# omerbt/TokenFlow

Hardware: NVIDIA H100
Metric: frames/sec for 40-frame 512x512 SD1.5 50-step edit (higher is better)
Workload: dtype fp16

## Files before the change

### tokenflow_b200/csrc/tf_nn_field.cu

```cuda
#include <cmath>

#include "tf_common.cuh"
#include "tf_kernels.h"
#include "tf_wgmma.cuh"

namespace tf {
namespace {

constexpr int kChunkK = 64;
constexpr int kBlockM = 128;
constexpr int kBlockN = 128;
constexpr int kMaxStages = 8;
constexpr int kSmemBudget = 227 * 1024;

struct NNItems {
  int32_t n_a;
  int32_t n_b;
  int32_t tiles_per_frame;
  int32_t n_b_frames;
  int32_t b_frames[kMaxFrames];
};

struct SmemCtl {
  uint64_t full[kMaxStages];
  uint64_t empty[kMaxStages];
  uint64_t a_full;
};

template <bool kResidentA>
__global__ void __launch_bounds__(288, 1)
nn_field_kernel(const __grid_constant__ CUtensorMap map_x, const __grid_constant__ CUtensorMap map_p,
                const FrameTable tab, const NNItems items, int S, int dim, int stages,
                int32_t* __restrict__ idx_a, int32_t* __restrict__ idx_b) {
  constexpr int kAChunkBytes = kBlockM * 128;
  constexpr int kBChunkBytes = kBlockN * 128;
  constexpr int kStageBytes = kBChunkBytes + (kResidentA ? 0 : kAChunkBytes);
  constexpr int kAcc = kBlockN / 2;

  extern __shared__ uint8_t smem_raw[];
  uint8_t* smem = reinterpret_cast<uint8_t*>((reinterpret_cast<uintptr_t>(smem_raw) + 1023) & ~uintptr_t(1023));
  const int nkc = (dim + kChunkK - 1) / kChunkK;
  uint8_t* a_res = smem;
  uint8_t* ring = smem + (kResidentA ? nkc * kAChunkBytes : 0);
  SmemCtl* ctl = reinterpret_cast<SmemCtl*>(ring + stages * kStageBytes);

  int f, m0, kf;
  int32_t* out;
  if ((int)blockIdx.x < items.n_a) {
    f = blockIdx.x / items.tiles_per_frame;
    m0 = (blockIdx.x - f * items.tiles_per_frame) * kBlockM;
    kf = tab.kf_a[f];
    out = idx_a;
  } else {
    const int j = blockIdx.x - items.n_a;
    const int fi = j / items.tiles_per_frame;
    f = items.b_frames[fi];
    m0 = (j - fi * items.tiles_per_frame) * kBlockM;
    kf = tab.kf_b[f];
    out = idx_b;
  }
  const int n_tiles = (S + kBlockN - 1) / kBlockN;
  const int J = n_tiles * nkc;

  auto load = [&](int j) {
    const int st = j % stages;
    const int nt = j / nkc, kc = j - nt * nkc;
    uint8_t* dst = ring + st * kStageBytes;
    mbar_arrive_expect_tx(&ctl->full[st], (uint32_t)kStageBytes);
    tma_load_3d(dst, &map_p, &ctl->full[st], kc * kChunkK, nt * kBlockN, kf);
    if (!kResidentA) tma_load_3d(dst + kBChunkBytes, &map_x, &ctl->full[st], kc * kChunkK, m0, f);
  };

  if (threadIdx.x == 0) {
    tma_prefetch_desc(&map_x);
    tma_prefetch_desc(&map_p);
    for (int i = 0; i < stages; ++i) {
      mbar_init(&ctl->full[i], 1);
      mbar_init(&ctl->empty[i], 8);
    }
    mbar_init(&ctl->a_full, 1);
    fence_mbar_init();
  }
  __syncthreads();
  if (threadIdx.x >= 256) {
    if (threadIdx.x == 256) {
      if (kResidentA) {
        mbar_arrive_expect_tx(&ctl->a_full, (uint32_t)(nkc * kAChunkBytes));
        for (int kc = 0; kc < nkc; ++kc) tma_load_3d(a_res + kc * kAChunkBytes, &map_x, &ctl->a_full, kc * kChunkK, m0, f);
      }
      for (int j = 0; j < J; ++j) {
        if (j >= stages) mbar_wait(&ctl->empty[j % stages], (uint32_t)(j / stages - 1) & 1u);
        load(j);
      }
    }
    return;
  }

  const int wg = threadIdx.x >> 7;
  const int lane = threadIdx.x & 31;
  const int qcol = 2 * (lane & 3);
  const uint32_t ring_addr = smem_u32(ring);
  const uint32_t a_res_addr = smem_u32(a_res) + wg * 64 * 128;
  if (kResidentA) {
    mbar_wait(&ctl->a_full, 0);
    __syncwarp();
  }

  auto release = [&](int j) {
    __syncwarp();
    if (lane == 0) mbar_arrive(&ctl->empty[j % stages]);
  };

  float best[2] = {-INFINITY, -INFINITY};
  int best_idx[2] = {0, 0};
  int j = 0;
  for (int nt = 0; nt < n_tiles; ++nt) {
    float acc[kAcc];
    for (int kc = 0; kc < nkc; ++kc, ++j) {
      const int st = j % stages;
      mbar_wait(&ctl->full[st], (uint32_t)(j / stages) & 1u);
      __syncwarp();
      const uint32_t b_addr = ring_addr + st * kStageBytes;
      const uint32_t a_addr = kResidentA ? a_res_addr + kc * kAChunkBytes : b_addr + kBChunkBytes + wg * 64 * 128;
      wgmma_fence();
#pragma unroll
      for (int k4 = 0; k4 < kChunkK / 16; ++k4)
        wgmma_ss<kBlockN>(acc, wgmma_desc(a_addr + k4 * 32, 16, 1024), wgmma_desc(b_addr + k4 * 32, 16, 1024),
                          (kc > 0 || k4 > 0) ? 1u : 0u);
      wgmma_commit();
      if (kc > 0) {
        wgmma_wait<1>();
        release(j - 1);
      }
    }
    wgmma_wait<0>();
    reg_fence(acc);
    release(j - 1);

    const int n0 = nt * kBlockN;
#pragma unroll
    for (int jb = 0; jb < kBlockN / 8; ++jb) {
#pragma unroll
      for (int e = 0; e < 4; ++e) {
        const int r = e >> 1;
        const int c = n0 + 8 * jb + qcol + (e & 1);
        const float h = __half2float(__float2half_rn(acc[4 * jb + e]));
        if (c < S && h > best[r]) { best[r] = h; best_idx[r] = c; }
      }
    }
  }

#pragma unroll
  for (int r = 0; r < 2; ++r) {
#pragma unroll
    for (int off = 1; off <= 2; off <<= 1) {
      const float ob = __shfl_xor_sync(0xffffffffu, best[r], off);
      const int oi = __shfl_xor_sync(0xffffffffu, best_idx[r], off);
      if (ob > best[r] || (ob == best[r] && oi < best_idx[r])) { best[r] = ob; best_idx[r] = oi; }
    }
    const int p = m0 + wg * 64 + ((threadIdx.x >> 5) & 3) * 16 + (lane >> 2) + 8 * r;
    if ((lane & 3) == 0 && p < S) out[(long long)f * S + p] = best_idx[r];
  }
}

template <bool kResidentA>
int launch_cfg(const void* x_unit, const void* piv_unit, const FrameTable& tab, const NNItems& items, int F, int S,
               int dim, int K, int32_t* idx_a, int32_t* idx_b, cudaStream_t stream) {
  const int nkc = (dim + kChunkK - 1) / kChunkK;
  const int a_bytes = kResidentA ? nkc * kBlockM * 128 : 0;
  const int stage_bytes = kBlockN * 128 + (kResidentA ? 0 : kBlockM * 128);
  int stages = (kSmemBudget - 2048 - a_bytes) / stage_bytes;
  if (stages > kMaxStages) stages = kMaxStages;
  if (stages < 2) {
    set_last_error("tf_nn_field: dim=%d does not fit the resident-A configuration", dim);
    return TF_ERR_UNSUPPORTED;
  }
  const size_t smem_bytes = 1024 + (size_t)a_bytes + (size_t)stages * stage_bytes + sizeof(SmemCtl);

  CUtensorMap map_x, map_p;
  {
    const uint64_t dims[3] = {(uint64_t)dim, (uint64_t)S, (uint64_t)F};
    const uint64_t strides[2] = {(uint64_t)dim * 2, (uint64_t)S * dim * 2};
    const uint32_t box[3] = {(uint32_t)kChunkK, (uint32_t)kBlockM, 1};
    CUresult r = encode_tiled(&map_x, CU_TENSOR_MAP_DATA_TYPE_FLOAT16, 3, x_unit, dims, strides, box,
                              CU_TENSOR_MAP_SWIZZLE_128B);
    if (r != CUDA_SUCCESS) { set_last_error("tf_nn_field: cuTensorMapEncodeTiled(x) failed: %d", (int)r); return TF_ERR_DRIVER; }
  }
  {
    const uint64_t dims[3] = {(uint64_t)dim, (uint64_t)S, (uint64_t)K};
    const uint64_t strides[2] = {(uint64_t)dim * 2, (uint64_t)S * dim * 2};
    const uint32_t box[3] = {(uint32_t)kChunkK, (uint32_t)kBlockN, 1};
    CUresult r = encode_tiled(&map_p, CU_TENSOR_MAP_DATA_TYPE_FLOAT16, 3, piv_unit, dims, strides, box,
                              CU_TENSOR_MAP_SWIZZLE_128B);
    if (r != CUDA_SUCCESS) { set_last_error("tf_nn_field: cuTensorMapEncodeTiled(pivots) failed: %d", (int)r); return TF_ERR_DRIVER; }
  }
  auto kern = nn_field_kernel<kResidentA>;
  if (check_cuda(cudaFuncSetAttribute(kern, cudaFuncAttributeMaxDynamicSharedMemorySize, (int)smem_bytes),
                 "tf_nn_field smem attribute"))
    return TF_ERR_CUDA;
  const int n_items = items.n_a + items.n_b;
  kern<<<n_items, 288, smem_bytes, stream>>>(map_x, map_p, tab, items, S, dim, stages, idx_a, idx_b);
  return check_cuda(cudaGetLastError(), "tf_nn_field launch");
}

}

int launch_nn_field(const void* x_unit, const void* piv_unit, const FrameTable& tab, int F, int S, int dim, int K,
                    int32_t* idx_a, int32_t* idx_b, cudaStream_t stream) {
  if (F == 0 || S == 0) return TF_OK;
  NNItems items;
  items.tiles_per_frame = (S + kBlockM - 1) / kBlockM;
  items.n_a = F * items.tiles_per_frame;
  items.n_b_frames = 0;
  for (int f = 0; f < F; ++f)
    if (tab.kf_b[f] >= 0) items.b_frames[items.n_b_frames++] = f;
  items.n_b = items.n_b_frames * items.tiles_per_frame;
  if (items.n_b > 0 && idx_b == nullptr) {
    set_last_error("tf_nn_field: idx_b is NULL but some frame has a second keyframe");
    return TF_ERR_INVALID_ARGUMENT;
  }
  if (dim <= 640) return launch_cfg<true>(x_unit, piv_unit, tab, items, F, S, dim, K, idx_a, idx_b, stream);
  return launch_cfg<false>(x_unit, piv_unit, tab, items, F, S, dim, K, idx_a, idx_b, stream);
}

}
```

### tokenflow_b200/csrc/tf_wgmma.cuh

```cuda
#pragma once

#include <stdint.h>

namespace tf {

template <int N> __device__ __forceinline__ void wgmma_ss(float (&d)[N / 2], uint64_t a, uint64_t b, uint32_t acc);
template <int N> __device__ __forceinline__ void wgmma_rs(float (&d)[N / 2], const uint32_t (&a)[4], uint64_t b, uint32_t acc);

template <>
__device__ __forceinline__ void wgmma_ss<64>(float (&d)[32], uint64_t a, uint64_t b, uint32_t acc) {
  asm volatile(
      "{\n\t.reg .pred p;\n\t"
      "setp.ne.b32 p, %34, 0;\n\t"
      "wgmma.mma_async.sync.aligned.m64n64k16.f32.f16.f16 "
      "{%0, %1, %2, %3, %4, %5, %6, %7, %8, %9, %10, %11, %12, %13, %14, %15, %16, %17, %18, %19, %20, %21, %22, %23, %24, %25, %26, %27, %28, %29, %30, %31}, "
      "%32, %33, p, 1, 1, 0, 0;\n\t}\n"
      : "+f"(d[0]), "+f"(d[1]), "+f"(d[2]), "+f"(d[3]), "+f"(d[4]), "+f"(d[5]), "+f"(d[6]), "+f"(d[7]),
        "+f"(d[8]), "+f"(d[9]), "+f"(d[10]), "+f"(d[11]), "+f"(d[12]), "+f"(d[13]), "+f"(d[14]), "+f"(d[15]),
        "+f"(d[16]), "+f"(d[17]), "+f"(d[18]), "+f"(d[19]), "+f"(d[20]), "+f"(d[21]), "+f"(d[22]), "+f"(d[23]),
        "+f"(d[24]), "+f"(d[25]), "+f"(d[26]), "+f"(d[27]), "+f"(d[28]), "+f"(d[29]), "+f"(d[30]), "+f"(d[31])
      : "l"(a), "l"(b), "r"(acc));
}

template <>
__device__ __forceinline__ void wgmma_ss<128>(float (&d)[64], uint64_t a, uint64_t b, uint32_t acc) {
  asm volatile(
      "{\n\t.reg .pred p;\n\t"
      "setp.ne.b32 p, %66, 0;\n\t"
      "wgmma.mma_async.sync.aligned.m64n128k16.f32.f16.f16 "
      "{%0, %1, %2, %3, %4, %5, %6, %7, %8, %9, %10, %11, %12, %13, %14, %15, %16, %17, %18, %19, %20, %21, %22, %23, %24, %25, %26, %27, %28, %29, %30, %31, %32, %33, %34, %35, %36, %37, %38, %39, %40, %41, %42, %43, %44, %45, %46, %47, %48, %49, %50, %51, %52, %53, %54, %55, %56, %57, %58, %59, %60, %61, %62, %63}, "
      "%64, %65, p, 1, 1, 0, 0;\n\t}\n"
      : "+f"(d[0]), "+f"(d[1]), "+f"(d[2]), "+f"(d[3]), "+f"(d[4]), "+f"(d[5]), "+f"(d[6]), "+f"(d[7]),
        "+f"(d[8]), "+f"(d[9]), "+f"(d[10]), "+f"(d[11]), "+f"(d[12]), "+f"(d[13]), "+f"(d[14]), "+f"(d[15]),
        "+f"(d[16]), "+f"(d[17]), "+f"(d[18]), "+f"(d[19]), "+f"(d[20]), "+f"(d[21]), "+f"(d[22]), "+f"(d[23]),
        "+f"(d[24]), "+f"(d[25]), "+f"(d[26]), "+f"(d[27]), "+f"(d[28]), "+f"(d[29]), "+f"(d[30]), "+f"(d[31]),
        "+f"(d[32]), "+f"(d[33]), "+f"(d[34]), "+f"(d[35]), "+f"(d[36]), "+f"(d[37]), "+f"(d[38]), "+f"(d[39]),
        "+f"(d[40]), "+f"(d[41]), "+f"(d[42]), "+f"(d[43]), "+f"(d[44]), "+f"(d[45]), "+f"(d[46]), "+f"(d[47]),
        "+f"(d[48]), "+f"(d[49]), "+f"(d[50]), "+f"(d[51]), "+f"(d[52]), "+f"(d[53]), "+f"(d[54]), "+f"(d[55]),
        "+f"(d[56]), "+f"(d[57]), "+f"(d[58]), "+f"(d[59]), "+f"(d[60]), "+f"(d[61]), "+f"(d[62]), "+f"(d[63])
      : "l"(a), "l"(b), "r"(acc));
}

template <>
__device__ __forceinline__ void wgmma_rs<16>(float (&d)[8], const uint32_t (&a)[4], uint64_t b, uint32_t acc) {
  asm volatile(
      "{\n\t.reg .pred p;\n\t"
      "setp.ne.b32 p, %13, 0;\n\t"
      "wgmma.mma_async.sync.aligned.m64n16k16.f32.f16.f16 "
      "{%0, %1, %2, %3, %4, %5, %6, %7}, "
      "{%8, %9, %10, %11}, %12, p, 1, 1, 1;\n\t}\n"
      : "+f"(d[0]), "+f"(d[1]), "+f"(d[2]), "+f"(d[3]), "+f"(d[4]), "+f"(d[5]), "+f"(d[6]), "+f"(d[7])
      : "r"(a[0]), "r"(a[1]), "r"(a[2]), "r"(a[3]), "l"(b), "r"(acc));
}

template <>
__device__ __forceinline__ void wgmma_rs<32>(float (&d)[16], const uint32_t (&a)[4], uint64_t b, uint32_t acc) {
  asm volatile(
      "{\n\t.reg .pred p;\n\t"
      "setp.ne.b32 p, %21, 0;\n\t"
      "wgmma.mma_async.sync.aligned.m64n32k16.f32.f16.f16 "
      "{%0, %1, %2, %3, %4, %5, %6, %7, %8, %9, %10, %11, %12, %13, %14, %15}, "
      "{%16, %17, %18, %19}, %20, p, 1, 1, 1;\n\t}\n"
      : "+f"(d[0]), "+f"(d[1]), "+f"(d[2]), "+f"(d[3]), "+f"(d[4]), "+f"(d[5]), "+f"(d[6]), "+f"(d[7]),
        "+f"(d[8]), "+f"(d[9]), "+f"(d[10]), "+f"(d[11]), "+f"(d[12]), "+f"(d[13]), "+f"(d[14]), "+f"(d[15])
      : "r"(a[0]), "r"(a[1]), "r"(a[2]), "r"(a[3]), "l"(b), "r"(acc));
}

template <>
__device__ __forceinline__ void wgmma_rs<48>(float (&d)[24], const uint32_t (&a)[4], uint64_t b, uint32_t acc) {
  asm volatile(
      "{\n\t.reg .pred p;\n\t"
      "setp.ne.b32 p, %29, 0;\n\t"
      "wgmma.mma_async.sync.aligned.m64n48k16.f32.f16.f16 "
      "{%0, %1, %2, %3, %4, %5, %6, %7, %8, %9, %10, %11, %12, %13, %14, %15, %16, %17, %18, %19, %20, %21, %22, %23}, "
      "{%24, %25, %26, %27}, %28, p, 1, 1, 1;\n\t}\n"
      : "+f"(d[0]), "+f"(d[1]), "+f"(d[2]), "+f"(d[3]), "+f"(d[4]), "+f"(d[5]), "+f"(d[6]), "+f"(d[7]),
        "+f"(d[8]), "+f"(d[9]), "+f"(d[10]), "+f"(d[11]), "+f"(d[12]), "+f"(d[13]), "+f"(d[14]), "+f"(d[15]),
        "+f"(d[16]), "+f"(d[17]), "+f"(d[18]), "+f"(d[19]), "+f"(d[20]), "+f"(d[21]), "+f"(d[22]), "+f"(d[23])
      : "r"(a[0]), "r"(a[1]), "r"(a[2]), "r"(a[3]), "l"(b), "r"(acc));
}

template <>
__device__ __forceinline__ void wgmma_rs<64>(float (&d)[32], const uint32_t (&a)[4], uint64_t b, uint32_t acc) {
  asm volatile(
      "{\n\t.reg .pred p;\n\t"
      "setp.ne.b32 p, %37, 0;\n\t"
      "wgmma.mma_async.sync.aligned.m64n64k16.f32.f16.f16 "
      "{%0, %1, %2, %3, %4, %5, %6, %7, %8, %9, %10, %11, %12, %13, %14, %15, %16, %17, %18, %19, %20, %21, %22, %23, %24, %25, %26, %27, %28, %29, %30, %31}, "
      "{%32, %33, %34, %35}, %36, p, 1, 1, 1;\n\t}\n"
      : "+f"(d[0]), "+f"(d[1]), "+f"(d[2]), "+f"(d[3]), "+f"(d[4]), "+f"(d[5]), "+f"(d[6]), "+f"(d[7]),
        "+f"(d[8]), "+f"(d[9]), "+f"(d[10]), "+f"(d[11]), "+f"(d[12]), "+f"(d[13]), "+f"(d[14]), "+f"(d[15]),
        "+f"(d[16]), "+f"(d[17]), "+f"(d[18]), "+f"(d[19]), "+f"(d[20]), "+f"(d[21]), "+f"(d[22]), "+f"(d[23]),
        "+f"(d[24]), "+f"(d[25]), "+f"(d[26]), "+f"(d[27]), "+f"(d[28]), "+f"(d[29]), "+f"(d[30]), "+f"(d[31])
      : "r"(a[0]), "r"(a[1]), "r"(a[2]), "r"(a[3]), "l"(b), "r"(acc));
}

template <>
__device__ __forceinline__ void wgmma_rs<80>(float (&d)[40], const uint32_t (&a)[4], uint64_t b, uint32_t acc) {
  asm volatile(
      "{\n\t.reg .pred p;\n\t"
      "setp.ne.b32 p, %45, 0;\n\t"
      "wgmma.mma_async.sync.aligned.m64n80k16.f32.f16.f16 "
      "{%0, %1, %2, %3, %4, %5, %6, %7, %8, %9, %10, %11, %12, %13, %14, %15, %16, %17, %18, %19, %20, %21, %22, %23, %24, %25, %26, %27, %28, %29, %30, %31, %32, %33, %34, %35, %36, %37, %38, %39}, "
      "{%40, %41, %42, %43}, %44, p, 1, 1, 1;\n\t}\n"
      : "+f"(d[0]), "+f"(d[1]), "+f"(d[2]), "+f"(d[3]), "+f"(d[4]), "+f"(d[5]), "+f"(d[6]), "+f"(d[7]),
        "+f"(d[8]), "+f"(d[9]), "+f"(d[10]), "+f"(d[11]), "+f"(d[12]), "+f"(d[13]), "+f"(d[14]), "+f"(d[15]),
        "+f"(d[16]), "+f"(d[17]), "+f"(d[18]), "+f"(d[19]), "+f"(d[20]), "+f"(d[21]), "+f"(d[22]), "+f"(d[23]),
        "+f"(d[24]), "+f"(d[25]), "+f"(d[26]), "+f"(d[27]), "+f"(d[28]), "+f"(d[29]), "+f"(d[30]), "+f"(d[31]),
        "+f"(d[32]), "+f"(d[33]), "+f"(d[34]), "+f"(d[35]), "+f"(d[36]), "+f"(d[37]), "+f"(d[38]), "+f"(d[39])
      : "r"(a[0]), "r"(a[1]), "r"(a[2]), "r"(a[3]), "l"(b), "r"(acc));
}

template <>
__device__ __forceinline__ void wgmma_rs<96>(float (&d)[48], const uint32_t (&a)[4], uint64_t b, uint32_t acc) {
  asm volatile(
      "{\n\t.reg .pred p;\n\t"
      "setp.ne.b32 p, %53, 0;\n\t"
      "wgmma.mma_async.sync.aligned.m64n96k16.f32.f16.f16 "
      "{%0, %1, %2, %3, %4, %5, %6, %7, %8, %9, %10, %11, %12, %13, %14, %15, %16, %17, %18, %19, %20, %21, %22, %23, %24, %25, %26, %27, %28, %29, %30, %31, %32, %33, %34, %35, %36, %37, %38, %39, %40, %41, %42, %43, %44, %45, %46, %47}, "
      "{%48, %49, %50, %51}, %52, p, 1, 1, 1;\n\t}\n"
      : "+f"(d[0]), "+f"(d[1]), "+f"(d[2]), "+f"(d[3]), "+f"(d[4]), "+f"(d[5]), "+f"(d[6]), "+f"(d[7]),
        "+f"(d[8]), "+f"(d[9]), "+f"(d[10]), "+f"(d[11]), "+f"(d[12]), "+f"(d[13]), "+f"(d[14]), "+f"(d[15]),
        "+f"(d[16]), "+f"(d[17]), "+f"(d[18]), "+f"(d[19]), "+f"(d[20]), "+f"(d[21]), "+f"(d[22]), "+f"(d[23]),
        "+f"(d[24]), "+f"(d[25]), "+f"(d[26]), "+f"(d[27]), "+f"(d[28]), "+f"(d[29]), "+f"(d[30]), "+f"(d[31]),
        "+f"(d[32]), "+f"(d[33]), "+f"(d[34]), "+f"(d[35]), "+f"(d[36]), "+f"(d[37]), "+f"(d[38]), "+f"(d[39]),
        "+f"(d[40]), "+f"(d[41]), "+f"(d[42]), "+f"(d[43]), "+f"(d[44]), "+f"(d[45]), "+f"(d[46]), "+f"(d[47])
      : "r"(a[0]), "r"(a[1]), "r"(a[2]), "r"(a[3]), "l"(b), "r"(acc));
}

template <>
__device__ __forceinline__ void wgmma_rs<112>(float (&d)[56], const uint32_t (&a)[4], uint64_t b, uint32_t acc) {
  asm volatile(
      "{\n\t.reg .pred p;\n\t"
      "setp.ne.b32 p, %61, 0;\n\t"
      "wgmma.mma_async.sync.aligned.m64n112k16.f32.f16.f16 "
      "{%0, %1, %2, %3, %4, %5, %6, %7, %8, %9, %10, %11, %12, %13, %14, %15, %16, %17, %18, %19, %20, %21, %22, %23, %24, %25, %26, %27, %28, %29, %30, %31, %32, %33, %34, %35, %36, %37, %38, %39, %40, %41, %42, %43, %44, %45, %46, %47, %48, %49, %50, %51, %52, %53, %54, %55}, "
      "{%56, %57, %58, %59}, %60, p, 1, 1, 1;\n\t}\n"
      : "+f"(d[0]), "+f"(d[1]), "+f"(d[2]), "+f"(d[3]), "+f"(d[4]), "+f"(d[5]), "+f"(d[6]), "+f"(d[7]),
        "+f"(d[8]), "+f"(d[9]), "+f"(d[10]), "+f"(d[11]), "+f"(d[12]), "+f"(d[13]), "+f"(d[14]), "+f"(d[15]),
        "+f"(d[16]), "+f"(d[17]), "+f"(d[18]), "+f"(d[19]), "+f"(d[20]), "+f"(d[21]), "+f"(d[22]), "+f"(d[23]),
        "+f"(d[24]), "+f"(d[25]), "+f"(d[26]), "+f"(d[27]), "+f"(d[28]), "+f"(d[29]), "+f"(d[30]), "+f"(d[31]),
        "+f"(d[32]), "+f"(d[33]), "+f"(d[34]), "+f"(d[35]), "+f"(d[36]), "+f"(d[37]), "+f"(d[38]), "+f"(d[39]),
        "+f"(d[40]), "+f"(d[41]), "+f"(d[42]), "+f"(d[43]), "+f"(d[44]), "+f"(d[45]), "+f"(d[46]), "+f"(d[47]),
        "+f"(d[48]), "+f"(d[49]), "+f"(d[50]), "+f"(d[51]), "+f"(d[52]), "+f"(d[53]), "+f"(d[54]), "+f"(d[55])
      : "r"(a[0]), "r"(a[1]), "r"(a[2]), "r"(a[3]), "l"(b), "r"(acc));
}

template <>
__device__ __forceinline__ void wgmma_rs<128>(float (&d)[64], const uint32_t (&a)[4], uint64_t b, uint32_t acc) {
  asm volatile(
      "{\n\t.reg .pred p;\n\t"
      "setp.ne.b32 p, %69, 0;\n\t"
      "wgmma.mma_async.sync.aligned.m64n128k16.f32.f16.f16 "
      "{%0, %1, %2, %3, %4, %5, %6, %7, %8, %9, %10, %11, %12, %13, %14, %15, %16, %17, %18, %19, %20, %21, %22, %23, %24, %25, %26, %27, %28, %29, %30, %31, %32, %33, %34, %35, %36, %37, %38, %39, %40, %41, %42, %43, %44, %45, %46, %47, %48, %49, %50, %51, %52, %53, %54, %55, %56, %57, %58, %59, %60, %61, %62, %63}, "
      "{%64, %65, %66, %67}, %68, p, 1, 1, 1;\n\t}\n"
      : "+f"(d[0]), "+f"(d[1]), "+f"(d[2]), "+f"(d[3]), "+f"(d[4]), "+f"(d[5]), "+f"(d[6]), "+f"(d[7]),
        "+f"(d[8]), "+f"(d[9]), "+f"(d[10]), "+f"(d[11]), "+f"(d[12]), "+f"(d[13]), "+f"(d[14]), "+f"(d[15]),
        "+f"(d[16]), "+f"(d[17]), "+f"(d[18]), "+f"(d[19]), "+f"(d[20]), "+f"(d[21]), "+f"(d[22]), "+f"(d[23]),
        "+f"(d[24]), "+f"(d[25]), "+f"(d[26]), "+f"(d[27]), "+f"(d[28]), "+f"(d[29]), "+f"(d[30]), "+f"(d[31]),
        "+f"(d[32]), "+f"(d[33]), "+f"(d[34]), "+f"(d[35]), "+f"(d[36]), "+f"(d[37]), "+f"(d[38]), "+f"(d[39]),
        "+f"(d[40]), "+f"(d[41]), "+f"(d[42]), "+f"(d[43]), "+f"(d[44]), "+f"(d[45]), "+f"(d[46]), "+f"(d[47]),
        "+f"(d[48]), "+f"(d[49]), "+f"(d[50]), "+f"(d[51]), "+f"(d[52]), "+f"(d[53]), "+f"(d[54]), "+f"(d[55]),
        "+f"(d[56]), "+f"(d[57]), "+f"(d[58]), "+f"(d[59]), "+f"(d[60]), "+f"(d[61]), "+f"(d[62]), "+f"(d[63])
      : "r"(a[0]), "r"(a[1]), "r"(a[2]), "r"(a[3]), "l"(b), "r"(acc));
}

template <>
__device__ __forceinline__ void wgmma_rs<144>(float (&d)[72], const uint32_t (&a)[4], uint64_t b, uint32_t acc) {
  asm volatile(
      "{\n\t.reg .pred p;\n\t"
      "setp.ne.b32 p, %77, 0;\n\t"
      "wgmma.mma_async.sync.aligned.m64n144k16.f32.f16.f16 "
      "{%0, %1, %2, %3, %4, %5, %6, %7, %8, %9, %10, %11, %12, %13, %14, %15, %16, %17, %18, %19, %20, %21, %22, %23, %24, %25, %26, %27, %28, %29, %30, %31, %32, %33, %34, %35, %36, %37, %38, %39, %40, %41, %42, %43, %44, %45, %46, %47, %48, %49, %50, %51, %52, %53, %54, %55, %56, %57, %58, %59, %60, %61, %62, %63, %64, %65, %66, %67, %68, %69, %70, %71}, "
      "{%72, %73, %74, %75}, %76, p, 1, 1, 1;\n\t}\n"
      : "+f"(d[0]), "+f"(d[1]), "+f"(d[2]), "+f"(d[3]), "+f"(d[4]), "+f"(d[5]), "+f"(d[6]), "+f"(d[7]),
        "+f"(d[8]), "+f"(d[9]), "+f"(d[10]), "+f"(d[11]), "+f"(d[12]), "+f"(d[13]), "+f"(d[14]), "+f"(d[15]),
        "+f"(d[16]), "+f"(d[17]), "+f"(d[18]), "+f"(d[19]), "+f"(d[20]), "+f"(d[21]), "+f"(d[22]), "+f"(d[23]),
        "+f"(d[24]), "+f"(d[25]), "+f"(d[26]), "+f"(d[27]), "+f"(d[28]), "+f"(d[29]), "+f"(d[30]), "+f"(d[31]),
        "+f"(d[32]), "+f"(d[33]), "+f"(d[34]), "+f"(d[35]), "+f"(d[36]), "+f"(d[37]), "+f"(d[38]), "+f"(d[39]),
        "+f"(d[40]), "+f"(d[41]), "+f"(d[42]), "+f"(d[43]), "+f"(d[44]), "+f"(d[45]), "+f"(d[46]), "+f"(d[47]),
        "+f"(d[48]), "+f"(d[49]), "+f"(d[50]), "+f"(d[51]), "+f"(d[52]), "+f"(d[53]), "+f"(d[54]), "+f"(d[55]),
        "+f"(d[56]), "+f"(d[57]), "+f"(d[58]), "+f"(d[59]), "+f"(d[60]), "+f"(d[61]), "+f"(d[62]), "+f"(d[63]),
        "+f"(d[64]), "+f"(d[65]), "+f"(d[66]), "+f"(d[67]), "+f"(d[68]), "+f"(d[69]), "+f"(d[70]), "+f"(d[71])
      : "r"(a[0]), "r"(a[1]), "r"(a[2]), "r"(a[3]), "l"(b), "r"(acc));
}

template <>
__device__ __forceinline__ void wgmma_rs<160>(float (&d)[80], const uint32_t (&a)[4], uint64_t b, uint32_t acc) {
  asm volatile(
      "{\n\t.reg .pred p;\n\t"
      "setp.ne.b32 p, %85, 0;\n\t"
      "wgmma.mma_async.sync.aligned.m64n160k16.f32.f16.f16 "
      "{%0, %1, %2, %3, %4, %5, %6, %7, %8, %9, %10, %11, %12, %13, %14, %15, %16, %17, %18, %19, %20, %21, %22, %23, %24, %25, %26, %27, %28, %29, %30, %31, %32, %33, %34, %35, %36, %37, %38, %39, %40, %41, %42, %43, %44, %45, %46, %47, %48, %49, %50, %51, %52, %53, %54, %55, %56, %57, %58, %59, %60, %61, %62, %63, %64, %65, %66, %67, %68, %69, %70, %71, %72, %73, %74, %75, %76, %77, %78, %79}, "
      "{%80, %81, %82, %83}, %84, p, 1, 1, 1;\n\t}\n"
      : "+f"(d[0]), "+f"(d[1]), "+f"(d[2]), "+f"(d[3]), "+f"(d[4]), "+f"(d[5]), "+f"(d[6]), "+f"(d[7]),
        "+f"(d[8]), "+f"(d[9]), "+f"(d[10]), "+f"(d[11]), "+f"(d[12]), "+f"(d[13]), "+f"(d[14]), "+f"(d[15]),
        "+f"(d[16]), "+f"(d[17]), "+f"(d[18]), "+f"(d[19]), "+f"(d[20]), "+f"(d[21]), "+f"(d[22]), "+f"(d[23]),
        "+f"(d[24]), "+f"(d[25]), "+f"(d[26]), "+f"(d[27]), "+f"(d[28]), "+f"(d[29]), "+f"(d[30]), "+f"(d[31]),
        "+f"(d[32]), "+f"(d[33]), "+f"(d[34]), "+f"(d[35]), "+f"(d[36]), "+f"(d[37]), "+f"(d[38]), "+f"(d[39]),
        "+f"(d[40]), "+f"(d[41]), "+f"(d[42]), "+f"(d[43]), "+f"(d[44]), "+f"(d[45]), "+f"(d[46]), "+f"(d[47]),
        "+f"(d[48]), "+f"(d[49]), "+f"(d[50]), "+f"(d[51]), "+f"(d[52]), "+f"(d[53]), "+f"(d[54]), "+f"(d[55]),
        "+f"(d[56]), "+f"(d[57]), "+f"(d[58]), "+f"(d[59]), "+f"(d[60]), "+f"(d[61]), "+f"(d[62]), "+f"(d[63]),
        "+f"(d[64]), "+f"(d[65]), "+f"(d[66]), "+f"(d[67]), "+f"(d[68]), "+f"(d[69]), "+f"(d[70]), "+f"(d[71]),
        "+f"(d[72]), "+f"(d[73]), "+f"(d[74]), "+f"(d[75]), "+f"(d[76]), "+f"(d[77]), "+f"(d[78]), "+f"(d[79])
      : "r"(a[0]), "r"(a[1]), "r"(a[2]), "r"(a[3]), "l"(b), "r"(acc));
}

template <>
__device__ __forceinline__ void wgmma_rs<176>(float (&d)[88], const uint32_t (&a)[4], uint64_t b, uint32_t acc) {
  asm volatile(
      "{\n\t.reg .pred p;\n\t"
      "setp.ne.b32 p, %93, 0;\n\t"
      "wgmma.mma_async.sync.aligned.m64n176k16.f32.f16.f16 "
      "{%0, %1, %2, %3, %4, %5, %6, %7, %8, %9, %10, %11, %12, %13, %14, %15, %16, %17, %18, %19, %20, %21, %22, %23, %24, %25, %26, %27, %28, %29, %30, %31, %32, %33, %34, %35, %36, %37, %38, %39, %40, %41, %42, %43, %44, %45, %46, %47, %48, %49, %50, %51, %52, %53, %54, %55, %56, %57, %58, %59, %60, %61, %62, %63, %64, %65, %66, %67, %68, %69, %70, %71, %72, %73, %74, %75, %76, %77, %78, %79, %80, %81, %82, %83, %84, %85, %86, %87}, "
      "{%88, %89, %90, %91}, %92, p, 1, 1, 1;\n\t}\n"
      : "+f"(d[0]), "+f"(d[1]), "+f"(d[2]), "+f"(d[3]), "+f"(d[4]), "+f"(d[5]), "+f"(d[6]), "+f"(d[7]),
        "+f"(d[8]), "+f"(d[9]), "+f"(d[10]), "+f"(d[11]), "+f"(d[12]), "+f"(d[13]), "+f"(d[14]), "+f"(d[15]),
        "+f"(d[16]), "+f"(d[17]), "+f"(d[18]), "+f"(d[19]), "+f"(d[20]), "+f"(d[21]), "+f"(d[22]), "+f"(d[23]),
        "+f"(d[24]), "+f"(d[25]), "+f"(d[26]), "+f"(d[27]), "+f"(d[28]), "+f"(d[29]), "+f"(d[30]), "+f"(d[31]),
        "+f"(d[32]), "+f"(d[33]), "+f"(d[34]), "+f"(d[35]), "+f"(d[36]), "+f"(d[37]), "+f"(d[38]), "+f"(d[39]),
        "+f"(d[40]), "+f"(d[41]), "+f"(d[42]), "+f"(d[43]), "+f"(d[44]), "+f"(d[45]), "+f"(d[46]), "+f"(d[47]),
        "+f"(d[48]), "+f"(d[49]), "+f"(d[50]), "+f"(d[51]), "+f"(d[52]), "+f"(d[53]), "+f"(d[54]), "+f"(d[55]),
        "+f"(d[56]), "+f"(d[57]), "+f"(d[58]), "+f"(d[59]), "+f"(d[60]), "+f"(d[61]), "+f"(d[62]), "+f"(d[63]),
        "+f"(d[64]), "+f"(d[65]), "+f"(d[66]), "+f"(d[67]), "+f"(d[68]), "+f"(d[69]), "+f"(d[70]), "+f"(d[71]),
        "+f"(d[72]), "+f"(d[73]), "+f"(d[74]), "+f"(d[75]), "+f"(d[76]), "+f"(d[77]), "+f"(d[78]), "+f"(d[79]),
        "+f"(d[80]), "+f"(d[81]), "+f"(d[82]), "+f"(d[83]), "+f"(d[84]), "+f"(d[85]), "+f"(d[86]), "+f"(d[87])
      : "r"(a[0]), "r"(a[1]), "r"(a[2]), "r"(a[3]), "l"(b), "r"(acc));
}

template <>
__device__ __forceinline__ void wgmma_rs<192>(float (&d)[96], const uint32_t (&a)[4], uint64_t b, uint32_t acc) {
  asm volatile(
      "{\n\t.reg .pred p;\n\t"
      "setp.ne.b32 p, %101, 0;\n\t"
      "wgmma.mma_async.sync.aligned.m64n192k16.f32.f16.f16 "
      "{%0, %1, %2, %3, %4, %5, %6, %7, %8, %9, %10, %11, %12, %13, %14, %15, %16, %17, %18, %19, %20, %21, %22, %23, %24, %25, %26, %27, %28, %29, %30, %31, %32, %33, %34, %35, %36, %37, %38, %39, %40, %41, %42, %43, %44, %45, %46, %47, %48, %49, %50, %51, %52, %53, %54, %55, %56, %57, %58, %59, %60, %61, %62, %63, %64, %65, %66, %67, %68, %69, %70, %71, %72, %73, %74, %75, %76, %77, %78, %79, %80, %81, %82, %83, %84, %85, %86, %87, %88, %89, %90, %91, %92, %93, %94, %95}, "
      "{%96, %97, %98, %99}, %100, p, 1, 1, 1;\n\t}\n"
      : "+f"(d[0]), "+f"(d[1]), "+f"(d[2]), "+f"(d[3]), "+f"(d[4]), "+f"(d[5]), "+f"(d[6]), "+f"(d[7]),
        "+f"(d[8]), "+f"(d[9]), "+f"(d[10]), "+f"(d[11]), "+f"(d[12]), "+f"(d[13]), "+f"(d[14]), "+f"(d[15]),
        "+f"(d[16]), "+f"(d[17]), "+f"(d[18]), "+f"(d[19]), "+f"(d[20]), "+f"(d[21]), "+f"(d[22]), "+f"(d[23]),
        "+f"(d[24]), "+f"(d[25]), "+f"(d[26]), "+f"(d[27]), "+f"(d[28]), "+f"(d[29]), "+f"(d[30]), "+f"(d[31]),
        "+f"(d[32]), "+f"(d[33]), "+f"(d[34]), "+f"(d[35]), "+f"(d[36]), "+f"(d[37]), "+f"(d[38]), "+f"(d[39]),
        "+f"(d[40]), "+f"(d[41]), "+f"(d[42]), "+f"(d[43]), "+f"(d[44]), "+f"(d[45]), "+f"(d[46]), "+f"(d[47]),
        "+f"(d[48]), "+f"(d[49]), "+f"(d[50]), "+f"(d[51]), "+f"(d[52]), "+f"(d[53]), "+f"(d[54]), "+f"(d[55]),
        "+f"(d[56]), "+f"(d[57]), "+f"(d[58]), "+f"(d[59]), "+f"(d[60]), "+f"(d[61]), "+f"(d[62]), "+f"(d[63]),
        "+f"(d[64]), "+f"(d[65]), "+f"(d[66]), "+f"(d[67]), "+f"(d[68]), "+f"(d[69]), "+f"(d[70]), "+f"(d[71]),
        "+f"(d[72]), "+f"(d[73]), "+f"(d[74]), "+f"(d[75]), "+f"(d[76]), "+f"(d[77]), "+f"(d[78]), "+f"(d[79]),
        "+f"(d[80]), "+f"(d[81]), "+f"(d[82]), "+f"(d[83]), "+f"(d[84]), "+f"(d[85]), "+f"(d[86]), "+f"(d[87]),
        "+f"(d[88]), "+f"(d[89]), "+f"(d[90]), "+f"(d[91]), "+f"(d[92]), "+f"(d[93]), "+f"(d[94]), "+f"(d[95])
      : "r"(a[0]), "r"(a[1]), "r"(a[2]), "r"(a[3]), "l"(b), "r"(acc));
}

}
```

Baseline: 2.913.

## Add register-resident A path and double-buffered accumulators to NN field kernel

For dims 258–320, the nearest-neighbour field kernel now keeps the first 256 columns of the query tile in registers and uses register-sourced wgmma, with only the fifth K chunk staged in shared memory. This frees shared memory for more pipeline stages. The other paths now ping-pong two accumulator sets so the argmax epilogue of one tile overlaps the MMAs of the next. Compile-time probe modes are added for timing experiments. The register path assumes exactly five K chunks and raises register pressure under the 288-thread, one-block-per-SM launch bound.

```diff
diff --git a/tokenflow_b200/csrc/tf_nn_field.cu b/tokenflow_b200/csrc/tf_nn_field.cu
--- a/tokenflow_b200/csrc/tf_nn_field.cu
+++ b/tokenflow_b200/csrc/tf_nn_field.cu
@@ -12,6 +12,11 @@
 constexpr int kBlockN = 128;
 constexpr int kMaxStages = 8;
 constexpr int kSmemBudget = 227 * 1024;
+
+#ifndef TF_NN_FIELD_PROBE
+#define TF_NN_FIELD_PROBE 0
+#endif
+constexpr int kProbe = TF_NN_FIELD_PROBE;
 
 struct NNItems {
   int32_t n_a;
@@ -27,39 +32,50 @@
   uint64_t a_full;
 };
 
-template <bool kResidentA>
+template <bool kResidentA, bool kRegA>
 __global__ void __launch_bounds__(288, 1)
 nn_field_kernel(const __grid_constant__ CUtensorMap map_x, const __grid_constant__ CUtensorMap map_p,
-                const FrameTable tab, const NNItems items, int S, int dim, int stages,
+                const __half* __restrict__ x, const FrameTable tab, const NNItems items, int S, int dim, int stages,
                 int32_t* __restrict__ idx_a, int32_t* __restrict__ idx_b) {
   constexpr int kAChunkBytes = kBlockM * 128;
   constexpr int kBChunkBytes = kBlockN * 128;
   constexpr int kStageBytes = kBChunkBytes + (kResidentA ? 0 : kAChunkBytes);
   constexpr int kAcc = kBlockN / 2;
+  constexpr int kRegNkc = kRegA ? 5 : 0;
+  constexpr int kRegChunks = 4;
+  constexpr bool kSmemA = kResidentA && !kRegA;
 
   extern __shared__ uint8_t smem_raw[];
   uint8_t* smem = reinterpret_cast<uint8_t*>((reinterpret_cast<uintptr_t>(smem_raw) + 1023) & ~uintptr_t(1023));
-  const int nkc = (dim + kChunkK - 1) / kChunkK;
+  const int nkc = kRegA ? kRegNkc : (dim + kChunkK - 1) / kChunkK;
   uint8_t* a_res = smem;
-  uint8_t* ring = smem + (kResidentA ? nkc * kAChunkBytes : 0);
+  uint8_t* ring = smem + (kSmemA ? nkc : kRegA ? kRegNkc - kRegChunks : 0) * kAChunkBytes;
   SmemCtl* ctl = reinterpret_cast<SmemCtl*>(ring + stages * kStageBytes);
 
   int f, m0, kf;
   int32_t* out;
-  if ((int)blockIdx.x < items.n_a) {
-    f = blockIdx.x / items.tiles_per_frame;
-    m0 = (blockIdx.x - f * items.tiles_per_frame) * kBlockM;
+  const int item = kProbe == 3 ? blockIdx.x >> 1 : blockIdx.x;
+  if (item < items.n_a) {
+    f = item / items.tiles_per_frame;
+    m0 = (item - f * items.tiles_per_frame) * kBlockM;
     kf = tab.kf_a[f];
     out = idx_a;
   } else {
-    const int j = blockIdx.x - items.n_a;
+    const int j = item - items.n_a;
     const int fi = j / items.tiles_per_frame;
     f = items.b_frames[fi];
     m0 = (j - fi * items.tiles_per_frame) * kBlockM;
     kf = tab.kf_b[f];
     out = idx_b;
   }
-  const int n_tiles = (S + kBlockN - 1) / kBlockN;
+  int n_tiles = (S + kBlockN - 1) / kBlockN;
+  int nt0 = 0;
+  if (kProbe == 3) {
+    const int half = (n_tiles + 1) / 2;
+    nt0 = (blockIdx.x & 1) * half;
+    n_tiles = min(half, n_tiles - nt0);
+    if (n_tiles <= 0) return;
+  }
   const int J = n_tiles * nkc;
 
   auto load = [&](int j) {
@@ -67,7 +83,7 @@
     const int nt = j / nkc, kc = j - nt * nkc;
     uint8_t* dst = ring + st * kStageBytes;
     mbar_arrive_expect_tx(&ctl->full[st], (uint32_t)kStageBytes);
-    tma_load_3d(dst, &map_p, &ctl->full[st], kc * kChunkK, nt * kBlockN, kf);
+    tma_load_3d(dst, &map_p, &ctl->full[st], kc * kChunkK, kProbe == 2 ? 0 : (nt0 + nt) * kBlockN, kf);
     if (!kResidentA) tma_load_3d(dst + kBChunkBytes, &map_x, &ctl->full[st], kc * kChunkK, m0, f);
   };
 
@@ -84,7 +100,11 @@
   __syncthreads();
   if (threadIdx.x >= 256) {
     if (threadIdx.x == 256) {
-      if (kResidentA) {
+      if (kRegA) {
+        mbar_arrive_expect_tx(&ctl->a_full, (uint32_t)kAChunkBytes);
+        tma_load_3d(a_res, &map_x, &ctl->a_full, kRegChunks * kChunkK, m0, f);
+      }
+      if (kSmemA) {
         mbar_arrive_expect_tx(&ctl->a_full, (uint32_t)(nkc * kAChunkBytes));
         for (int kc = 0; kc < nkc; ++kc) tma_load_3d(a_res + kc * kAChunkBytes, &map_x, &ctl->a_full, kc * kChunkK, m0, f);
       }
@@ -101,9 +121,22 @@
   const int qcol = 2 * (lane & 3);
   const uint32_t ring_addr = smem_u32(ring);
   const uint32_t a_res_addr = smem_u32(a_res) + wg * 64 * 128;
-  if (kResidentA) {
+  if (kSmemA || kRegA) {
     mbar_wait(&ctl->a_full, 0);
     __syncwarp();
+  }
+  uint32_t afrag[kRegA ? kRegChunks * 4 : 1][4];
+  if (kRegA) {
+    const int r = m0 + wg * 64 + ((threadIdx.x >> 5) & 3) * 16 + (lane >> 2);
+#pragma unroll
+    for (int ks = 0; ks < kRegChunks * 4; ++ks)
+#pragma unroll
+      for (int i = 0; i < 4; ++i) {
+        const int row = r + 8 * (i & 1);
+        const int k = ks * 16 + qcol + 8 * (i >> 1);
+        afrag[ks][i] = (row < S && k < dim)
+                           ? *reinterpret_cast<const uint32_t*>(x + ((long long)f * S + row) * dim + k) : 0u;
+      }
   }
 
   auto release = [&](int j) {
@@ -113,31 +146,13 @@
 
   float best[2] = {-INFINITY, -INFINITY};
   int best_idx[2] = {0, 0};
-  int j = 0;
-  for (int nt = 0; nt < n_tiles; ++nt) {
-    float acc[kAcc];
-    for (int kc = 0; kc < nkc; ++kc, ++j) {
-      const int st = j % stages;
-      mbar_wait(&ctl->full[st], (uint32_t)(j / stages) & 1u);
-      __syncwarp();
-      const uint32_t b_addr = ring_addr + st * kStageBytes;
-      const uint32_t a_addr = kResidentA ? a_res_addr + kc * kAChunkBytes : b_addr + kBChunkBytes + wg * 64 * 128;
-      wgmma_fence();
-#pragma unroll
-      for (int k4 = 0; k4 < kChunkK / 16; ++k4)
-        wgmma_ss<kBlockN>(acc, wgmma_desc(a_addr + k4 * 32, 16, 1024), wgmma_desc(b_addr + k4 * 32, 16, 1024),
-                          (kc > 0 || k4 > 0) ? 1u : 0u);
-      wgmma_commit();
-      if (kc > 0) {
-        wgmma_wait<1>();
-        release(j - 1);
-      }
-    }
-    wgmma_wait<0>();
-    reg_fence(acc);
-    release(j - 1);
-
-    const int n0 = nt * kBlockN;
+
+  auto epilogue = [&](float (&acc)[kAcc], int nt) {
+    if (kProbe == 1) {
+      best[0] = fmaxf(best[0], acc[0]);
+      return;
+    }
+    const int n0 = (nt0 + nt) * kBlockN;
 #pragma unroll
     for (int jb = 0; jb < kBlockN / 8; ++jb) {
 #pragma unroll
@@ -148,6 +163,80 @@
         if (c < S && h > best[r]) { best[r] = h; best_idx[r] = c; }
       }
     }
+  };
+
+  int j = 0;
+  auto chunk = [&](float (&acc)[kAcc], int kc) {
+    const int st = j % stages;
+    mbar_wait(&ctl->full[st], (uint32_t)(j / stages) & 1u);
+    __syncwarp();
+    const uint32_t b_addr = ring_addr + st * kStageBytes;
+    const uint32_t a_addr = kRegA ? a_res_addr : kResidentA ? a_res_addr + kc * kAChunkBytes
+                                                            : b_addr + kBChunkBytes + wg * 64 * 128;
+    wgmma_fence();
+#pragma unroll
+    for (int k4 = 0; k4 < kChunkK / 16; ++k4) {
+      if (kRegA && kc < kRegChunks)
+        wgmma_rs_kmajor<kBlockN>(acc, afrag[kRegA && kc < kRegChunks ? kc * 4 + k4 : 0], wgmma_desc(b_addr + k4 * 32, 16, 1024),
+                                 (kc > 0 || k4 > 0) ? 1u : 0u);
+      else
+        wgmma_ss<kBlockN>(acc, wgmma_desc(a_addr + k4 * 32, 16, 1024), wgmma_desc(b_addr + k4 * 32, 16, 1024),
+                          (kc > 0 || k4 > 0) ? 1u : 0u);
+    }
+    wgmma_commit();
+  };
+  auto retire = [&]() {
+    wgmma_wait<1>();
+    if (j > 0) release(j - 1);
+    ++j;
+  };
+  if constexpr (kRegA) {
+    float acc[kAcc];
+    for (int nt = 0; nt < n_tiles; ++nt) {
+#pragma unroll
+      for (int kc = 0; kc < kRegNkc; ++kc) {
+        chunk(acc, kc);
+        if (kc > 0) {
+          wgmma_wait<1>();
+          release(j - 1);
+        }
+        ++j;
+      }
+      wgmma_wait<0>();
+      reg_fence(acc);
+      release(j - 1);
+      epilogue(acc, nt);
+    }
+  } else {
+  auto mma_tile = [&](float (&acc)[kAcc], float (&prev)[kAcc], int nt) {
+    chunk(acc, 0);
+    retire();
+    if (nkc > 1) chunk(acc, 1);
+    reg_fence(prev);
+    epilogue(prev, nt - 1);
+    if (nkc > 1) retire();
+#pragma unroll
+    for (int kc = 2; kc < (kRegA ? kRegNkc : nkc); ++kc) {
+      chunk(acc, kc);
+      retire();
+    }
+  };
+  float acc0[kAcc], acc1[kAcc];
+#pragma unroll
+  for (int i = 0; i < kAcc; ++i) acc1[i] = -INFINITY;
+  for (int nt = 0; nt < n_tiles; nt += 2) {
+    mma_tile(acc0, acc1, nt);
+    if (nt + 1 < n_tiles) mma_tile(acc1, acc0, nt + 1);
+  }
+  wgmma_wait<0>();
+  release(j - 1);
+  if (n_tiles & 1) {
+    reg_fence(acc0);
+    epilogue(acc0, n_tiles - 1);
+  } else {
+    reg_fence(acc1);
+    epilogue(acc1, n_tiles - 1);
+  }
   }
 
 #pragma unroll
@@ -163,11 +252,11 @@
   }
 }
 
-template <bool kResidentA>
+template <bool kResidentA, bool kRegA>
 int launch_cfg(const void* x_unit, const void* piv_unit, const FrameTable& tab, const NNItems& items, int F, int S,
                int dim, int K, int32_t* idx_a, int32_t* idx_b, cudaStream_t stream) {
   const int nkc = (dim + kChunkK - 1) / kChunkK;
-  const int a_bytes = kResidentA ? nkc * kBlockM * 128 : 0;
+  const int a_bytes = (kRegA ? 1 : kResidentA ? nkc : 0) * kBlockM * 128;
   const int stage_bytes = kBlockN * 128 + (kResidentA ? 0 : kBlockM * 128);
   int stages = (kSmemBudget - 2048 - a_bytes) / stage_bytes;
   if (stages > kMaxStages) stages = kMaxStages;
@@ -194,12 +283,13 @@
                               CU_TENSOR_MAP_SWIZZLE_128B);
     if (r != CUDA_SUCCESS) { set_last_error("tf_nn_field: cuTensorMapEncodeTiled(pivots) failed: %d", (int)r); return TF_ERR_DRIVER; }
   }
-  auto kern = nn_field_kernel<kResidentA>;
+  auto kern = nn_field_kernel<kResidentA, kRegA>;
   if (check_cuda(cudaFuncSetAttribute(kern, cudaFuncAttributeMaxDynamicSharedMemorySize, (int)smem_bytes),
                  "tf_nn_field smem attribute"))
     return TF_ERR_CUDA;
-  const int n_items = items.n_a + items.n_b;
-  kern<<<n_items, 288, smem_bytes, stream>>>(map_x, map_p, tab, items, S, dim, stages, idx_a, idx_b);
+  const int n_items = (items.n_a + items.n_b) * (kProbe == 3 ? 2 : 1);
+  kern<<<n_items, 288, smem_bytes, stream>>>(map_x, map_p, static_cast<const __half*>(x_unit), tab, items, S, dim,
+                                             stages, idx_a, idx_b);
   return check_cuda(cudaGetLastError(), "tf_nn_field launch");
 }
 
@@ -219,8 +309,10 @@
     set_last_error("tf_nn_field: idx_b is NULL but some frame has a second keyframe");
     return TF_ERR_INVALID_ARGUMENT;
   }
-  if (dim <= 640) return launch_cfg<true>(x_unit, piv_unit, tab, items, F, S, dim, K, idx_a, idx_b, stream);
-  return launch_cfg<false>(x_unit, piv_unit, tab, items, F, S, dim, K, idx_a, idx_b, stream);
-}
-
-}
+  if (dim > 256 && dim <= 320 && dim % 2 == 0)
+    return launch_cfg<true, true>(x_unit, piv_unit, tab, items, F, S, dim, K, idx_a, idx_b, stream);
+  if (dim <= 640) return launch_cfg<true, false>(x_unit, piv_unit, tab, items, F, S, dim, K, idx_a, idx_b, stream);
+  return launch_cfg<false, false>(x_unit, piv_unit, tab, items, F, S, dim, K, idx_a, idx_b, stream);
+}
+
+}
diff --git a/tokenflow_b200/csrc/tf_wgmma.cuh b/tokenflow_b200/csrc/tf_wgmma.cuh
--- a/tokenflow_b200/csrc/tf_wgmma.cuh
+++ b/tokenflow_b200/csrc/tf_wgmma.cuh
@@ -39,6 +39,28 @@
         "+f"(d[48]), "+f"(d[49]), "+f"(d[50]), "+f"(d[51]), "+f"(d[52]), "+f"(d[53]), "+f"(d[54]), "+f"(d[55]),
         "+f"(d[56]), "+f"(d[57]), "+f"(d[58]), "+f"(d[59]), "+f"(d[60]), "+f"(d[61]), "+f"(d[62]), "+f"(d[63])
       : "l"(a), "l"(b), "r"(acc));
+}
+
+template <int N> __device__ __forceinline__ void wgmma_rs_kmajor(float (&d)[N / 2], const uint32_t (&a)[4], uint64_t b,
+                                                                 uint32_t acc);
+
+template <>
+__device__ __forceinline__ void wgmma_rs_kmajor<128>(float (&d)[64], const uint32_t (&a)[4], uint64_t b, uint32_t acc) {
+  asm volatile(
+      "{\n\t.reg .pred p;\n\t"
+      "setp.ne.b32 p, %69, 0;\n\t"
+      "wgmma.mma_async.sync.aligned.m64n128k16.f32.f16.f16 "
+      "{%0, %1, %2, %3, %4, %5, %6, %7, %8, %9, %10, %11, %12, %13, %14, %15, %16, %17, %18, %19, %20, %21, %22, %23, %24, %25, %26, %27, %28, %29, %30, %31, %32, %33, %34, %35, %36, %37, %38, %39, %40, %41, %42, %43, %44, %45, %46, %47, %48, %49, %50, %51, %52, %53, %54, %55, %56, %57, %58, %59, %60, %61, %62, %63}, "
+      "{%64, %65, %66, %67}, %68, p, 1, 1, 0;\n\t}\n"
+      : "+f"(d[0]), "+f"(d[1]), "+f"(d[2]), "+f"(d[3]), "+f"(d[4]), "+f"(d[5]), "+f"(d[6]), "+f"(d[7]),
+        "+f"(d[8]), "+f"(d[9]), "+f"(d[10]), "+f"(d[11]), "+f"(d[12]), "+f"(d[13]), "+f"(d[14]), "+f"(d[15]),
+        "+f"(d[16]), "+f"(d[17]), "+f"(d[18]), "+f"(d[19]), "+f"(d[20]), "+f"(d[21]), "+f"(d[22]), "+f"(d[23]),
+        "+f"(d[24]), "+f"(d[25]), "+f"(d[26]), "+f"(d[27]), "+f"(d[28]), "+f"(d[29]), "+f"(d[30]), "+f"(d[31]),
+        "+f"(d[32]), "+f"(d[33]), "+f"(d[34]), "+f"(d[35]), "+f"(d[36]), "+f"(d[37]), "+f"(d[38]), "+f"(d[39]),
+        "+f"(d[40]), "+f"(d[41]), "+f"(d[42]), "+f"(d[43]), "+f"(d[44]), "+f"(d[45]), "+f"(d[46]), "+f"(d[47]),
+        "+f"(d[48]), "+f"(d[49]), "+f"(d[50]), "+f"(d[51]), "+f"(d[52]), "+f"(d[53]), "+f"(d[54]), "+f"(d[55]),
+        "+f"(d[56]), "+f"(d[57]), "+f"(d[58]), "+f"(d[59]), "+f"(d[60]), "+f"(d[61]), "+f"(d[62]), "+f"(d[63])
+      : "r"(a[0]), "r"(a[1]), "r"(a[2]), "r"(a[3]), "l"(b), "r"(acc));
 }
 
 template <>
```

New measurement: 2.933 (median of 6 runs). No clear change (+0.7%).
